# riktor/safer2-recommender

Hardware: AMD Instinct MI355X
Metric: user-solve updates/sec + sec/epoch, iALS dim=256 ml20m-shaped (higher is better)
Workload: dtype f32

## Files before the change

safer2-recommender_amd/csrc/capi.hip:

```cpp
#include <hip/hip_runtime.h>
#include <rccl/rccl.h>

#include <algorithm>
#include <climits>
#include <cmath>
#include <cstdio>
#include <cstdlib>
#include <cstring>
#include <map>
#include <random>
#include <string>
#include <thread>
#include <vector>

#include "ctx.h"
#include "wide.h"

namespace {
std::string g_last_error;
}

namespace frecsys_hip {

int fail(frecsys_ctx* c, int code, const std::string& msg) {
// ... 560 lines not shown
  if (Dp == 0)
    return fail(nullptr, FRECSYS_ERR_UNSUPPORTED,
                "dim " + std::to_string(cfg->dim) + " not supported (1..1024 built)");
  if (cfg->n_users < 0 || cfg->n_items < 0)
    return fail(nullptr, FRECSYS_ERR_INVALID, "negative entity counts");
  int cnt = 0;
  if (hipGetDeviceCount(&cnt) != hipSuccess || cnt == 0)
    return fail(nullptr, FRECSYS_ERR_NO_DEVICE, "no HIP device visible");
  auto* c = new frecsys_ctx();
  c->dim = cfg->dim;
  c->Dp = Dp;
  c->quirks = cfg->parity_quirks;
  c->n[0] = cfg->n_users;
  c->n[1] = cfg->n_items;
  if (cfg->device >= 0) {
    c->device = cfg->device;
  } else {
    (void)hipGetDevice(&c->device);
  }
  auto bail = [&](int rc) {
    g_last_error = c->err;
    frecsys_ctx_destroy(c);
    return rc;
  };
  if (hipSetDevice(c->device) != hipSuccess)
    return bail(fail(c, FRECSYS_ERR_NO_DEVICE, "hipSetDevice failed"));
  {
    int lo_pri = 0, hi_pri = 0;
    (void)hipDeviceGetStreamPriorityRange(&lo_pri, &hi_pri);
    if (hipStreamCreateWithPriority(&c->stream.h, hipStreamNonBlocking, hi_pri) != hipSuccess)
      return bail(fail(c, FRECSYS_ERR_HIP, "hipStreamCreate failed"));
  }
  if (hipEventCreate(&c->ev0.h) != hipSuccess || hipEventCreate(&c->ev1.h) != hipSuccess)
    return bail(fail(c, FRECSYS_ERR_HIP, "hipEventCreate failed"));
  const int s3_pri = 0;
  if (hipStreamCreateWithFlags(&c->stream2.h, hipStreamNonBlocking) != hipSuccess ||
      hipStreamCreateWithPriority(&c->stream3.h, hipStreamNonBlocking, s3_pri) != hipSuccess ||
      hipEventCreateWithFlags(&c->ev_fork.h, hipEventDisableTiming) != hipSuccess ||
      hipEventCreateWithFlags(&c->ev_join.h, hipEventDisableTiming) != hipSuccess ||
      hipEventCreateWithFlags(&c->ev_fork3.h, hipEventDisableTiming) != hipSuccess ||
      hipEventCreateWithFlags(&c->ev_join3.h, hipEventDisableTiming) != hipSuccess)
    return bail(fail(c, FRECSYS_ERR_HIP, "hipStreamCreate failed (stream2/3)"));
  c->stream5 = c->stream3.h;
  if (hipEventCreateWithFlags(&c->ev_pre5.h, hipEventDisableTiming) != hipSuccess ||
      hipEventCreateWithFlags(&c->ev_eager[0].h, hipEventDisableTiming) != hipSuccess ||
      hipEventCreateWithFlags(&c->ev_eager[1].h, hipEventDisableTiming) != hipSuccess)
    return bail(fail(c, FRECSYS_ERR_HIP, "hipEventCreate failed (early builds)"));
  if (const char* v = getenv("FRECSYS_DUAL")) c->dual_on = atoi(v);
  if (const char* v = getenv("FRECSYS_EAGER")) c->eager_on = atoi(v);
  if (const char* v = getenv("FRECSYS_CHOL_BASIS")) c->chol_basis_on = atoi(v);
  c->dual_max_h = Dp <= 256 ? 224 : Dp == 1024 ? 512 : 256;
  if (const char* v = getenv("FRECSYS_DUAL_MAX_H")) c->dual_max_h = atoi(v);
  if (const char* v = getenv("FRECSYS_DUAL_SERIAL")) c->dual_serial = atoi(v);
  if (const char* v = getenv("FRECSYS_SPLIT_ROWS")) c->split_rows = atoi(v);
  if (const char* v = getenv("FRECSYS_DEBUG_SKIP")) {
#ifdef FRECSYS_ABLATION
    c->debug_skip = atoi(v);
#else
    if (atoi(v) != 0)
      return bail(fail(c, FRECSYS_ERR_INVALID,
                       "FRECSYS_DEBUG_SKIP needs a -DFRECSYS_ABLATION build of libfrecsys_hip.so"));
#endif
  }
  if (const char* v = getenv("FRECSYS_WIDE_WS_MB")) c->wide_ws_mb = std::max(1, atoi(v));
  if (const char* v = getenv("FRECSYS_WIDE_PRESPLIT")) c->wide_presplit = atoi(v) != 0;
  if (const char* v = getenv("FRECSYS_WS_FREE_CAP")) c->ws_free_cap = atoi(v) != 0;
  const int max_h_cap = Dp >= 512 ? kDualWideMaxH : 32 * kDualMaxTiles;
  c->dual_max_h = std::min(c->dual_max_h, max_h_cap);
  for (int t = 0; t < 3; ++t) c->dual_max_h_side[t] = c->dual_max_h;
  if (Dp == 512 && !getenv("FRECSYS_DUAL_MAX_H"))
    c->dual_max_h_side[FRECSYS_SIDE_USER] = std::min(320, max_h_cap);
  if (const char* v = getenv("FRECSYS_DUAL_MAX_H_USER"))
    c->dual_max_h_side[0] = std::min(atoi(v), max_h_cap);
  if (const char* v = getenv("FRECSYS_DUAL_MAX_H_ITEM"))
    c->dual_max_h_side[1] = std::min(atoi(v), max_h_cap);
  for (int s = 0; s < 2; ++s) {
    const size_t rows = (size_t)std::max<int64_t>(c->n[s], 1);
    if (c->emb[s].reserve(rows * Dp) != hipSuccess ||
        c->gram[s].reserve((size_t)Dp * Dp) != hipSuccess)
      return bail(fail(c, FRECSYS_ERR_HIP, "hipMalloc failed (embeddings)"));
    (void)hipMemsetAsync(c->emb[s], 0, sizeof(float) * rows * Dp, c->stream);
    (void)hipMemsetAsync(c->gram[s], 0, sizeof(float) * Dp * Dp, c->stream);
  }
  if (c->d_fail.reserve(1) != hipSuccess || c->d_counter.reserve(1) != hipSuccess ||
      c->d_events.reserve(4) != hipSuccess)
    return bail(fail(c, FRECSYS_ERR_HIP, "hipMalloc failed"));
  (void)hipMemsetAsync(c->d_events, 0, 4 * sizeof(unsigned int), c->stream);
  c->bounds[0] = {0, c->n[0]};
  c->bounds[1] = {0, c->n[1]};
  if (hipStreamSynchronize(c->stream) != hipSuccess)
    return bail(fail(c, FRECSYS_ERR_HIP, "stream sync failed"));
  *out = c;
  return FRECSYS_OK;
}

void frecsys_ctx_destroy(frecsys_ctx* c) {
  if (!c) return;
  (void)hipSetDevice(c->device);
  for (hipStream_t s : {c->stream5, c->stream.h, c->stream2.h})
    if (s) (void)hipStreamSynchronize(s);
  if (c->comm) ncclCommDestroy(c->comm);
  delete c;
}

int frecsys_comm_unique_id(uint8_t id[128]) {
  ncclUniqueId uid;
// ... 605 lines not shown
```

safer2-recommender_amd/csrc/chol.h:

```cpp
#pragma once

#include "common.h"

constexpr int kCholYWave = 4;
constexpr int kCholWPrio = 1;

namespace frecsys_hip {

__device__ __forceinline__ float rdlane(float v, int l) {
  return __int_as_float(__builtin_amdgcn_readlane(__float_as_int(v), l));
}

typedef __attribute__((address_space(3))) float lds_float;

template <int G>
__device__ __forceinline__ void load_factor_rows(const lds_float* tile, int r, bool fl,
                                                 float (&a)[32]) {
  typedef __attribute__((address_space(3))) const f32x4v lds_f32x4c;
#pragma unroll
  for (int g = 0; g < 8; ++g) {
    const f32x4v v = *reinterpret_cast<lds_f32x4c*>(tile + r * 32 + (((g ^ (r >> 1)) & 7) << 2));
#pragma unroll
    for (int t = 0; t < 4; ++t) a[4 * g + t] = v[t];
  }
  if constexpr (G == 1) {
#pragma unroll
    for (int c = 0; c < 32; ++c) asm volatile("" : "+v"(a[c]));
  }
#pragma unroll
  for (int c = 0; c < 32; ++c) a[c] = fl ? a[c] : (c == r ? 1.0f : 0.0f);
}

__device__ __forceinline__ bool diag_factor_inv_lds_body(lds_float* tile, int lane) {
  const int r = lane & 31;
  const bool fl = lane < 32;
  float a[32];
  load_factor_rows<1>(tile, r, fl, a);
  int pmin = 0x7fffffff, pmax = 0;
#pragma unroll
  for (int k = 0; k < 32; ++k) {
    float p0 = 0.f, p1 = 0.f, p2 = 0.f, p3 = 0.f;
#pragma unroll
    for (int m = 0; m < k; m += 4) {
      const float b0 = rdlane(a[m], k);
      const float b1 = m + 1 < k ? rdlane(a[m + 1], k) : 0.0f;
      const float b2 = m + 2 < k ? rdlane(a[m + 2], k) : 0.0f;
      const float b3 = m + 3 < k ? rdlane(a[m + 3], k) : 0.0f;
      p0 += a[m] * b0;
      if (m + 1 < k) p1 += a[m + 1] * b1;
      if (m + 2 < k) p2 += a[m + 2] * b2;
      if (m + 3 < k) p3 += a[m + 3] * b3;
    }
    const float t = a[k] - ((p0 + p1) + (p2 + p3));
    const float piv = rdlane(t, k);
    const int pi = __builtin_amdgcn_readfirstlane(__float_as_int(piv));
// ... 302 lines not shown
      if (hi == 0) xvec[32 * p + lo] = x;
    }
    lds_barrier();
  }
}

typedef __attribute__((address_space(3))) int lds_int;

__device__ __forceinline__ int ld_ver(const int* f) {
  return __builtin_amdgcn_readfirstlane(*(volatile lds_int*)(f));
}
__device__ __forceinline__ void wait_ver(const int* f, int v) {
  if (ld_ver(f) < v) {
    do {
      __builtin_amdgcn_s_sleep(1);
    } while (ld_ver(f) < v);
  }
  asm volatile("" ::: "memory");
}
__device__ __forceinline__ void set_ver(int* f, int v, int lane) {
  asm volatile("s_waitcnt lgkmcnt(0)" ::: "memory");
  if (lane == 0) *(volatile lds_int*)(f) = v;
  asm volatile("" ::: "memory");
}

template <bool TR>
__device__ __forceinline__ float tile_gemv(const float* M, const float* v, int lo, int hi) {
  float s0 = 0.0f, s1 = 0.0f;
  if constexpr (!TR) {
#pragma unroll
    for (int g = 0; g < 4; ++g) {
      const f32x4v x = row_gran(M, lo, 4 * hi + g);
      const int m0 = 16 * hi + 4 * g;
      s0 += x[0] * v[m0];
      s1 += x[1] * v[m0 + 1];
      s0 += x[2] * v[m0 + 2];
      s1 += x[3] * v[m0 + 3];
    }
  } else {
#pragma unroll
    for (int m = 0; m < 16; m += 2) {
      const int m0 = 16 * hi + m;
      s0 += M[TR ? sw(m0, lo) : sw(lo, m0)] * v[m0];
      s1 += M[TR ? sw(m0 + 1, lo) : sw(lo, m0 + 1)] * v[m0 + 1];
    }
  }
  const float s = s0 + s1;
  return s + __shfl_xor(s, 32);
}

template <int T, int NW, bool BLK = true>
__device__ __forceinline__ void chol_solve_df(float* tiles, float* bvec, float* xvec,
                                              float* part, int* flag, int tid, int debug_skip,
                                              unsigned long long* prof = nullptr) {
  static_assert(NW >= 2, "one chain wave and at least one worker");
  constexpr int NT = T * (T + 1) / 2;
  constexpr bool X6 = BLK;
  constexpr bool FUSE = BLK;
  const unsigned long long t0 = prof ? clock64() : 0;
  const int lane = tid & 63, lo = lane & 31, hi = lane >> 5;
  const int wave = __builtin_amdgcn_readfirstlane(tid >> 6);
  int* ver = reinterpret_cast<int*>(part);
  int* bver = ver + NT;
  int* rcnt = bver + T;
  int* yver = rcnt + T;
  int* xver = yver + 1;
  float* rbuf = part + ((NT + 2 * T + 2 + 3) & ~3);
  if (tid < NT + 2 * T + 2) ver[tid] = 0;
  lds_barrier();

  auto trsm = [&](int I, int p) {
    float* Aip = tiles + tidx(I, p) * 1024;
    if (!FRECSYS_SKIP(debug_skip, 4)) {
      const f32x16 u = X6 ? tile_pqT_x6(Aip, tiles + tidx(p, p) * 1024, lo, hi)
                          : tile_pqT(Aip, tiles + tidx(p, p) * 1024, lo, hi);
#pragma unroll
      for (int q = 0; q < 16; ++q) Aip[sw(acc_row(q, hi), lo)] = u[q];
    }
    set_ver(ver + tidx(I, p), p + 1, lane);
  };
  auto bupd = [&](int I, int p) {
    wait_ver(bver + I, p);
    const float t = tile_gemv<false>(tiles + tidx(I, p) * 1024, bvec + 32 * p, lo, hi);
    if (hi == 0) bvec[32 * I + lo] -= t;
    set_ver(bver + I, p + 1, lane);
  };
  auto update = [&](int I, int J, int p) {
    float* Aij = tiles + tidx(I, J) * 1024;
    if (!FRECSYS_SKIP(debug_skip, 8)) {
      const float* Li = tiles + tidx(I, p) * 1024;
      const float* Lj = tiles + tidx(J, p) * 1024;
      const f32x16 u = !X6     ? tile_pqT(Li, Lj, lo, hi)
                       : I == J ? tile_pqT_x6<true>(Li, Li, lo, hi)
                                : tile_pqT_x6(Li, Lj, lo, hi);
#pragma unroll
      for (int q = 0; q < 16; ++q) Aij[sw(acc_row(q, hi), lo)] -= u[q];
    }
    set_ver(ver + tidx(I, J), p + 1, lane);
  };
  auto factor = [&](int p) {
    float* Tpp = tiles + tidx(p, p) * 1024;
    if (!FRECSYS_SKIP(debug_skip, 2)) {
      if (!diag_factor_inv<BLK>(Tpp, lane) && lane == 0) flag[0] = 1;
    }
    set_ver(ver + tidx(p, p), p + 1, lane);
  };
  auto ysolve = [&](int p) {
// ... 29 lines not shown
          if (!YW) bupd(p + 1, p);
          lap(ts);
          wait_ver(ver + tidx(p + 1, p + 1), p);
          lap(tw);
          const float* Lnp = tiles + tidx(p + 1, p) * 1024;
          f32x16 u = f32x16{0.f};
          if (!FRECSYS_SKIP(debug_skip, 8)) u = tile_pqT_x6<true>(Lnp, Lnp, lo, hi);
#pragma unroll
          for (int q = 0; q < 16; ++q) u[q] = Tnn[sw(acc_row(q, hi), lo)] - u[q];
          lap(tu);
          if (!FRECSYS_SKIP(debug_skip, 2)) ok = diag_factor_inv_acc(u, (lds_float*)Tnn);
        } else {
          if (!FRECSYS_SKIP(debug_skip, 2)) ok = diag_factor_inv_blk((lds_float*)Tnn, lane);
        }
        if (!ok && lane == 0) flag[0] = 1;
        set_ver(ver + tidx(p + 1, p + 1), p + 2, lane);
      } else {
        if (p >= 0) {
          wait_ver(ver + tidx(p + 1, p), p);
          lap(tw);
          trsm(p + 1, p);
          if (!YW) bupd(p + 1, p);
          lap(ts);
          wait_ver(ver + tidx(p + 1, p + 1), p);
          lap(tw);
          update(p + 1, p + 1, p);
          lap(tu);
        }
        factor(p + 1);
      }
      if (!YW) ysolve(p + 1);
      lap(tf);
    }
    if (prof && lane == 0) {
      atomicAdd(prof + 11, tw);
      atomicAdd(prof + 12, ts);
      atomicAdd(prof + 13, tu);
      atomicAdd(prof + 14, tf);
    }
    __builtin_amdgcn_s_setprio(0);
    if (prof && lane == 0) atomicAdd(prof + 5, clock64() - t0);
  } else if (YW && wave == YWAVE) {
#pragma unroll 1
    for (int p = 0; p < T; ++p) {
      wait_ver(ver + tidx(p, p), p + 1);
      wait_ver(bver + p, p);
      ysolve(p);
      if (p + 1 < T) {
        wait_ver(ver + tidx(p + 1, p), p + 1);
        bupd(p + 1, p);
      }
    }
  } else {
    int k = 0;
    unsigned long long tww = 0;
    auto wwait = [&](const int* f, int v) {
      if (prof) {
        const unsigned long long t = clock64();
        wait_ver(f, v);
        tww += clock64() - t;
      } else {
        wait_ver(f, v);
      }
    };
    auto wprio = [&](bool c) {
      if (c) __builtin_amdgcn_s_setprio(1);
      else __builtin_amdgcn_s_setprio(0);
    };
#pragma unroll 1
    for (int p = 0; p + 1 < T; ++p) {
#pragma unroll 1
      for (int I = p + 2; I < T; ++I, ++k) {
        if (wk_wave(k % NWK) != wave) continue;
        wwait(ver + tidx(p, p), p + 1);
        wwait(ver + tidx(I, p), p);
        wprio(I <= p + 1 + kCholWPrio);
        trsm(I, p);
        wwait(yver, p + 1);
        bupd(I, p);
      }
#pragma unroll 1
      for (int J = p + 1; J < T; ++J) {
#pragma unroll 1
        for (int I = (J == p + 1 ? p + 2 : J); I < T; ++I, ++k) {
          if (wk_wave(k % NWK) != wave) continue;
          wwait(ver + tidx(I, p), p + 1);
          wwait(ver + tidx(J, p), p + 1);
          wwait(ver + tidx(I, J), p);
          wprio(I <= p + 1 + kCholWPrio);
          update(I, J, p);
        }
      }
    }
    __builtin_amdgcn_s_setprio(0);
    if (prof && lane == 0) {
      atomicAdd(prof + 6, (clock64() - t0) / NWK);
      atomicAdd(prof + 15, tww / NWK);
    }
  }
  lds_barrier();
  if (prof && tid == 0) atomicAdd(prof + 7, clock64() - t0);

  if (wave == 0) {
    __builtin_amdgcn_s_setprio(2);
#pragma unroll 1
    for (int p = T - 1; p >= 0; --p) {
      float r = bvec[32 * p + lo];
      if (p + 1 < T) {
        wait_ver(rcnt + p, T - 2 - p);
        r = bvec[32 * p + lo] -
            tile_gemv<true>(tiles + tidx(p + 1, p) * 1024, xvec + 32 * (p + 1), lo, hi);
      }
      if (hi == 0) rbuf[lo] = r;
      wave_lds_sync();
      const float x = tile_gemv<true>(tiles + tidx(p, p) * 1024, rbuf, lo, hi);
      if (hi == 0) xvec[32 * p + lo] = x;
      set_ver(xver, T - p, lane);
    }
    __builtin_amdgcn_s_setprio(0);
  } else {
#pragma unroll 1
    for (int q = T - 1; q >= 2; --q) {
#pragma unroll 1
      for (int p = 0; p + 2 <= q; ++p) {
        if (1 + p % (NW - 1) != wave) continue;
        wait_ver(xver, T - q);
        const float t = tile_gemv<true>(tiles + tidx(q, p) * 1024, xvec + 32 * q, lo, hi);
        if (hi == 0) bvec[32 * p + lo] -= t;
        set_ver(rcnt + p, T - q, lane);
      }
    }
  }
  lds_barrier();
}

}
```

safer2-recommender_amd/csrc/ctx.h:

```cpp
#pragma once

#include <hip/hip_runtime.h>
#include <rccl/rccl.h>

#include <cstdint>
#include <map>
#include <string>
#include <vector>

#include "../../include/frecsys_hip.h"
#include "device_buf.h"
#include "kernels.h"

namespace frecsys_hip {

struct Timer {
  double total_ms = 0.0;
  int64_t launches = 0;
};

struct Work {
  double flops = 0.0, bytes = 0.0;
  int64_t entities = 0, launches = 0;
};
// ... 80 lines not shown
  std::vector<int32_t> cg_bstart;
  std::vector<int32_t> cg_iters[3];
  int64_t cg_iterations = 0, cg_unconverged = 0;
  DevBuf<float> wide_ws;
  DevBuf<char> wide_xs;
  DevBuf<char> dw_zs;
  DevBuf<float> dw_slots;
  DevBuf<float> dw_z;
  bool wide_presplit = true;
  int64_t wide_ws_mb = 16384;
  bool ws_free_cap = true;
  int64_t ws_shrinks = 0;
  int split_rows = 4096;
  std::vector<int2> h_split;
  std::vector<SplitWork> h_work;
  DevBuf<int2> d_split;
  DevBuf<SplitWork> d_work;
  DevBuf<float> d_slabs;
  std::vector<int32_t> order_h[3];
  std::vector<QueueRec> h_order[3];
  int dual_on = 1;
  uint64_t ver_counter = 0;
  uint64_t emb_ver[3] = {0, 0, 0};
  uint64_t gram_ver[2] = {0, 0};
  uint64_t gram_src[2] = {0, 0};
  uint64_t basis_gram[2] = {0, 0};
  uint64_t xrot_emb[2] = {0, 0};
  uint64_t xrot_gram[2] = {0, 0};
  uint64_t xrot_sub[2] = {0, 0};
  DevBuf<QueueRec> d_hrows[3];
  int64_t n_hrows[3] = {-1, -1, -1};
  int64_t hrows_key[3][2] = {{-1, -1}, {-1, -1}, {-1, -1}};
  struct WorkPrefix {
    bool valid = false;
    std::vector<double> h1, h2, h3;
    std::vector<int64_t> nz;
  };
  WorkPrefix wprefix[3][2];
  uint64_t hrows_gen[3] = {0, 0, 0};
  DevBuf<uint8_t> d_mark;
  bool dual_used[3] = {false, false, false};
  int eager_on = 1;
  int basis_mode[2] = {0, 0};
  float basis_mu[2] = {0.f, 0.f}, basis_lam[2] = {0.f, 0.f};
  int want_mode[2] = {0, 0};
  float want_mu[2] = {0.f, 0.f}, want_lam[2] = {0.f, 0.f};
  int chol_basis_on = 1;
  DevBuf<float> chol_work;
  bool eager_pending[2] = {false, false};
  int dual_max_h = 256;
  int dual_max_h_side[3] = {256, 256, 256};
  int dual_serial = 0;
  int debug_skip = 0;
  struct Pending {
    std::string name;
    hipEvent_t a, b;
  };
  std::vector<Pending> pending;
  std::vector<hipEvent_t> event_pool;
};

namespace frecsys_hip {

int fail(frecsys_ctx* c, int code, const std::string& msg);

#define HIP_TRY(c, expr)                                                            \
  do {                                                                              \
    hipError_t _e = (expr);                                                         \
    if (_e != hipSuccess)                                                           \
      return fail((c), FRECSYS_ERR_HIP,                                             \
                  std::string(#expr) + ": " + hipGetErrorString(_e));               \
  } while (0)

#define NCCL_TRY(c, expr)                                                           \
  do {                                                                              \
    ncclResult_t _r = (expr);                                                       \
    if (_r != ncclSuccess)                                                          \
      return fail((c), FRECSYS_ERR_RCCL,                                            \
                  std::string(#expr) + ": " + ncclGetErrorString(_r));              \
  } while (0)

void add_work(frecsys_ctx* c, const std::string& key, double flops, double bytes,
              int64_t entities);

void partition_rows(int64_t n_rows, const int64_t* row_ptr, int parts, int64_t* bounds);

template <typename T>
int ensure(frecsys_ctx* c, DevBuf<T>& b, size_t count) {
  const hipError_t e = b.reserve(count);
  if (e == hipSuccess) return FRECSYS_OK;
  return fail(c, FRECSYS_ERR_HIP,
              std::string(b ? "hipFree(*p): "
                            : "hipMalloc((void**)p, sizeof(T) * std::max<size_t>(count, 1)): ") +
                  hipGetErrorString(e));
}

#pragma GCC visibility push(hidden)

template <typename T>
int try_ensure(frecsys_ctx* c, DevBuf<T>& b, size_t count, bool* oom) {
  const hipError_t e = b.try_reserve(count, oom);
  if (e == hipSuccess) return FRECSYS_OK;
  return fail(c, FRECSYS_ERR_HIP,
              std::string(b ? "hipFree(*p): " : "hipMalloc: ") + hipGetErrorString(e));
}

// ... 82 lines not shown
```

safer2-recommender_amd/csrc/dual.hip:

```cpp
#include <hip/hip_runtime.h>

#include <cstdlib>
#include <type_traits>

#include "chol.h"
#include "common.h"
#include "kernels.h"

namespace frecsys_hip {

namespace {

constexpr int kMaxDp = 1024;

template <int HP>
__device__ __forceinline__ int dgran(int p, int g, int hh, int j) {
  return ((p * 2 + g) * 2 + hh) * HP + j;
}

template <int TH, bool BF>
struct DualCfg {
  static constexpr int HP = 32 * TH;
  static constexpr int NT = TH * (TH + 1) / 2;
  static constexpr int NW = (TH <= 4) ? 4 : 8;
// ... 314 lines not shown
        const bf16x8* zb = reinterpret_cast<const bf16x8*>(zs);
#pragma unroll
        for (int m = 0; m < MT; ++m) {
          if (valid[m]) {
#pragma unroll
            for (int g = 0; g < 2; ++g) {
              bf16x8 av[3], bv[3];
#pragma unroll
              for (int p = 0; p < 3; ++p) {
                av[p] = zb[dgran<HP>(p, g, hi, aoff[m])];
                bv[p] = zb[dgran<HP>(p, g, hi, boff[m])];
              }
              acc[m] = mfma_x6(av, bv, acc[m]);
            }
          }
        }
      } else {
#pragma unroll
        for (int m = 0; m < MT; ++m) {
          if (valid[m]) {
#pragma unroll
            for (int s = 0; s < 16; ++s) {
              const float* zr = zs + (2 * s + hi) * HP;
              acc[m] = mfma32(zr[aoff[m]], zr[boff[m]], acc[m]);
            }
          }
        }
      }
    }
    if (!RDS && c + 1 < NC) store_slab(next, (c + 1) & 1);
    lds_barrier();
  };
  for (int c = 0; c < NC; c += 2) {
    slab_step(c, ra, rb);
    if (c + 1 < NC) slab_step(c + 1, rb, ra);
  }

#pragma unroll
  for (int m = 0; m < MT; ++m) {
    if (valid[m]) {
      const int I = (aoff[m] - lo) >> 5, J = (boff[m] - lo) >> 5;
      float* tile = tiles + tidx(I, J) * 1024;
#pragma unroll
      for (int q = 0; q < 16; ++q) {
        const int i = acc_row(q, hi);
        const bool dg = (32 * I + i) == (32 * J + lo);
        tile[sw(i, lo)] = acc[m][q] + (dg ? 1.0f : 0.0f);
      }
    }
  }
  lds_barrier();
  mark(1);
  chol_solve_df<TH, NW, (TH >= kDualBlkTH)>(tiles, bvec, xvec, part, flag, tid, a.debug_skip,
                                            a.prof);
  mark(2);

  {
    const int D4 = Dp >> 2, R = NTHR / D4;
    const int c4 = tid % D4, g = tid / D4;
    float* red = tiles;
    float4 acc4 = make_float4(0.f, 0.f, 0.f, 0.f);
    if (g < R && !FRECSYS_SKIP(a.debug_skip, 64)) {
      for (int j0 = g; j0 < ntot; j0 += 8 * R) {
        float4 rv[8];
        float wv[8];
#pragma unroll
        for (int u = 0; u < 8; ++u) {
          const int j = j0 + u * R;
          rv[u] = make_float4(0.f, 0.f, 0.f, 0.f);
          wv[u] = 0.0f;
          if (j < ntot) {
            wv[u] = cvec[j] * xvec[j];
            rv[u] = *reinterpret_cast<const float4*>(a.Xrot + (int64_t)ids[j] * Dp + 4 * c4);
          }
        }
#pragma unroll
        for (int u = 0; u < 8; ++u) {
          acc4.x += wv[u] * rv[u].x;
          acc4.y += wv[u] * rv[u].y;
          acc4.z += wv[u] * rv[u].z;
          acc4.w += wv[u] * rv[u].w;
        }
      }
      *reinterpret_cast<float4*>(red + g * Dp + 4 * c4) = acc4;
    }
    lds_barrier();
    for (int i = tid; i < Dp; i += NTHR) {
      float v = 0.0f;
      for (int gg = 0; gg < R; ++gg) v += red[gg * Dp + i];
      a.out_rot[blk_v(a.pos0 + blockIdx.x, i, Dp)] = v;
    }
  }
  mark(3);
  if (a.prof && tid == 0) atomicAdd(a.prof + 4, 1ull);
  if (tid == 0 && flag[0]) atomicMin(a.fail, (unsigned long long)(e + 1));
}


__device__ __forceinline__ void wave_sync() { wave_lds_sync(); }

template <int T>
__device__ __forceinline__ void chol_solve_wave(float* tiles, float* bvec, float* xvec,
                                                int* flag, int lane, int debug_skip) {
  const int lo = lane & 31, hi = lane >> 5;
  float y[T];
#pragma unroll
  for (int p = 0; p < T; ++p) {
// ... 710 lines not shown
```

safer2-recommender_amd/csrc/kernels.h:

```cpp
#pragma once

#include <hip/hip_runtime.h>
#include <stdint.h>

#include <vector>

namespace frecsys_hip {

struct QueueRec {
  int32_t entity;
  int32_t h;
  int64_t p0;
};

struct SplitWork {
  int32_t pos;
  int32_t k0;
  int32_t k1;
  int32_t slab;
};

struct SolveArgs {
  int kind;
  int quirk;
  const int64_t* row_ptr;
  const int32_t* col;
  int64_t row_lo;
  int64_t n_rows;
  const QueueRec* order;
  unsigned int* counter;
  const float* X;
  int64_t n_other;
  const float* G;
  const float* E;
  float* out;
  float reg, reg_exp, w, alpha, eta;
  int lambda_is_reg;
  const float* entity_weight;
  const float* entity_reg;
  const float* other_weight;
  unsigned long long* fail;
  int debug_skip;
  unsigned long long* prof;
  const int2* split;
  int64_t n_split;
  float* slabs;
  const SplitWork* work;
  int64_t n_work;
  const char* xsplit;
};

constexpr int kGramGroups = 16;
struct GramPlan {
  int64_t n = 0;
  int64_t rpl = 0;
  int64_t nleaf = 0;
  int ngroup = 0;
  size_t slab_floats = 0;
};
GramPlan gram_plan(int Dp, int64_t n);
inline int64_t gram_group_leaf(const GramPlan& p, int g) {
  return p.ngroup ? (int64_t)g * p.nleaf / p.ngroup : 0;
}
inline void gram_owned_groups(const GramPlan& p, int world, int rank, int* lo, int* hi) {
  *lo = (int)((int64_t)p.ngroup * rank / world);
  *hi = (int)((int64_t)p.ngroup * (rank + 1) / world);
}
size_t gram_leaf_floats(const GramPlan& p, int g_lo, int g_hi);

struct GramArgs {
  const float* X;
  const float* w;
  float* partials;
  float* gslabs;
  GramPlan plan;
  int g_lo, g_hi;
  int64_t row0;
  int64_t n;
};

struct LossArgs {
  const int64_t* row_ptr;
  const int32_t* col;
  int64_t row_lo, n_rows;
  const float* U;
  const float* V;
  const float* G;
  float beta;
  int half;
  float* out;
  float* quad;
  int quad_parts;
  void* gsplit;
  int raw;
  hipEvent_t ev_gather;
};


struct DualArgs {
  int kind;
  int quirk;
  int Dp;
  const QueueRec* order;
  int64_t n_rows;
  const int32_t* col;
  const float* Xrot;
  const float* tdiag;
  const float* toff;
  int unit_m;
  const float* basis_status;
  int64_t n_other;
  float* out_rot;
  float* table;
  int64_t pos0;
  float reg, reg_exp, w, alpha;
  int lambda_is_reg;
  const float* entity_weight;
  const float* entity_reg;
  const float* other_weight;
  unsigned long long* fail;
  int debug_skip;
  unsigned long long* prof;
};

constexpr int kDualMaxTiles = 8;

constexpr int kCgE = 16;
constexpr int kCgU = 8;
constexpr int kCgCoopRows = 256;
constexpr int kCgBatchRows = 4096;
struct CgArgs {
  int kind;
  int quirk;
  int Dp, dim;
  const QueueRec* order;
  const int32_t* bstart;
  int64_t n_batches;
  const int32_t* col;
  const float* X;
  int64_t n_other;
  const float* G;
  float* out;
  float reg, reg_exp, w, alpha;
  int lambda_is_reg;
  const float* entity_weight;
  const float* entity_reg;
  const float* other_weight;
  int max_iter;
  float tol;
  int32_t* iters;
  unsigned long long* stats;
  unsigned long long* fail;
};
size_t cg_lds_bytes(int Dp);
void cg_plan_batches(const QueueRec* order, int64_t n, std::vector<int32_t>* bstart);
hipError_t launch_cg(const CgArgs& a, hipStream_t s);

constexpr int kExplainGroup = 32;
constexpr int kExplainChunk = 256;
constexpr int kExplainMaxTop = 32;
struct ExplainArgs {
  int kind;
  int Dp;
  const int64_t* row_ptr;
  const int32_t* col;
  const int64_t* qrows;
  int64_t r0, n;
  const int64_t* tgt_ptr;
  const int32_t* tgt;
  int64_t tgt_base;
  const int64_t* coff;
  const int32_t* prow;
  const int32_t* order;
  const float* X;
// ... 273 lines not shown
```

safer2-recommender_amd/csrc/solve.hip:

```cpp
#include <hip/hip_runtime.h>

#include <type_traits>

#include "chol.h"
#include "common.h"
#include "kernels.h"

constexpr int kSyrkSB = 1;

namespace frecsys_hip {

namespace {

constexpr int kRing = 4;

template <int T, bool BF>
struct TiledCfg {
  static constexpr int Dp = 32 * T;
  static constexpr int NT = T * (T + 1) / 2;
  static constexpr int NW = (T <= 2) ? 4 : 8;
  static constexpr int NTHR = NW * 64;
  static constexpr int MT = (NT + NW - 1) / NW;
  static constexpr int R = BF ? 32 : ((T <= 2) ? 16 : (T >= 8 ? 64 : 32));
  static constexpr int NSLOT = R * Dp / 4;
// ... 508 lines not shown
          }
        }
      }
      if (tid < Dp) {
#pragma unroll 4
        for (int r = 0; r < R; ++r) bacc += ring_bw[slot * R + r] * st[r * Dp + tid];
      }
      if (more) store_stage(buf ^ 1, c + 1);
      if (ring_more) ring_store(c + 2, nid, nsa, nbw);
      lds_barrier();
    }
    store_tiles();
  }
  mark(1);
  if constexpr (BF) {
    if (bown && bg == 1) part[bc] = bpart;
    lds_barrier();
    if (tid < Dp) bacc += bpart + part[tid];
    lds_barrier();
  }
  mark(9);

  if (PARTIAL) {
    if (tid < Dp) a.slabs[(size_t)slab0 * slab_floats + NT * 1024 + tid] = bacc;
    return;
  }

  mark(10);
  if (tid < Dp) {
    float b = bacc;
    if (is_u_kind(kind)) b *= us;
    bvec[tid] = b;
  }
  lds_barrier();
  mark(2);

  if (grad) {
    if (tid < Dp) {
      const int i = tid, I = i >> 5, ri = i & 31;
      float y = 0.0f;
      for (int j = 0; j < Dp; ++j) {
        float aij;
        if (j <= i)
          aij = tiles[tidx(I, j >> 5) * 1024 + sw(ri, j & 31)];
        else
          aij = cvar_upper(kind, a.G[i * Dp + j], a.w, omega);
        y += aij * xvec[j];
      }
      a.out[e * Dp + i] = xvec[i] - a.eta * (y - bvec[i]);
    }
    return;
  }

  chol_solve_df<T, NW>(tiles, bvec, xvec, part, flag, tid, a.debug_skip, a.prof);
  mark(3);
  if (tid < Dp) a.out[e * Dp + tid] = xvec[tid];
  if (tid == 0 && flag[0]) atomicMin(a.fail, (unsigned long long)(e + 1));
  if (a.prof && tid == 0) {
    atomicAdd(a.prof + 4, 1ull);
    atomicAdd(a.prof + 8, (unsigned long long)ntot);
  }
}

__device__ __forceinline__ void wave_sync() {
  __builtin_amdgcn_fence(__ATOMIC_RELEASE, "wavefront");
  __builtin_amdgcn_wave_barrier();
  __builtin_amdgcn_fence(__ATOMIC_ACQUIRE, "wavefront");
}

template <int Dp>
__global__ void __launch_bounds__(256) solve_small_kernel(SolveArgs a) {
  constexpr int WPB = 4, CH = 64, PER = Dp * Dp / 64;
  __shared__ float sA[WPB][Dp * Dp];
  __shared__ float sX[WPB][CH * Dp];
  __shared__ float sB[WPB][Dp];
  __shared__ float sE[WPB][Dp];
  __shared__ float sSA[WPB][CH];
  __shared__ float sBW[WPB][CH];
  const int wave = threadIdx.x >> 6, lane = threadIdx.x & 63;
  const int64_t idx = (int64_t)blockIdx.x * WPB + wave;
  if (idx >= a.n_rows) return;
  const int64_t e = a.row_lo + idx;
  const int64_t p0 = a.row_ptr[e];
  const int64_t h = a.row_ptr[e + 1] - p0;
  if (h == 0) return;
  const int kind = a.kind;
  const bool vk = is_v_kind(kind);
  int64_t extra = 0;
  if (vk && a.quirk && h > 128 && (h % 128) != 0) extra = 128 - (h % 128);
  const int64_t ntot = h + extra;
  float acc[PER];
#pragma unroll
  for (int t = 0; t < PER; ++t) acc[t] = 0.0f;
  float bacc = 0.0f;
  float* X = sX[wave];
  for (int64_t c0 = 0; c0 < ntot; c0 += CH) {
    const int64_t k = c0 + lane;
    int id = -1;
    float sa = 0.f, bw = 0.f;
    if (k < ntot) {
      id = a.col[p0 + virt_pos(k, h)];
      if (vk) {
        const float nu = a.other_weight[id];
        sa = sqrtf(nu);
        bw = (k < h) ? nu : 0.0f;
      } else {
        sa = 1.0f;
// ... 209 lines not shown
```

safer2-recommender_amd/csrc/train.hip:

```cpp
#include <algorithm>
#include <climits>
#include <cstdio>
#include <cstdlib>
#include <string>
#include <vector>

#include "ctx.h"
#include "wide.h"

namespace {

const char* const kSolveNames[3] = {"solve_user", "solve_item", "solve_eval"};

bool is_vkind(int kind) { return kind == FRECSYS_KIND_WEIGHTED_V || kind == FRECSYS_KIND_CVAR_GRAD_V; }
bool is_ukind(int kind) { return kind == FRECSYS_KIND_WEIGHTED_U || kind == FRECSYS_KIND_CVAR_GRAD_U; }
bool is_grad(int kind) { return kind == FRECSYS_KIND_CVAR_GRAD_U || kind == FRECSYS_KIND_CVAR_GRAD_V; }

double dspace_solve_flops(double d) { return d * d * d / 3.0 + 2.0 * d * d; }

bool dual_prof_on() {
  static const bool on = getenv("FRECSYS_DUAL_PROF") != nullptr;
  return on;
}
int prof_counters(frecsys_ctx* c, DevBuf<unsigned long long>& buf, size_t n,
// ... 229 lines not shown
  }
  if (is_vkind(p->kind)) {
    rc = upload(c, c->d_entity_reg, p->entity_reg, (size_t)c->n[side]);
    if (rc) return rc;
    rc = upload(c, c->d_other_weight, p->other_weight, (size_t)c->n[other]);
    if (rc) return rc;
  }
  HIP_TRY(c, hipMemsetAsync(c->d_fail, 0xFF, sizeof(unsigned long long), c->stream));
  return FRECSYS_OK;
}

int end_solve(frecsys_ctx* c, int side, bool gather, unsigned long long* f) {
  HIP_TRY(c, hipMemcpyAsync(f, c->d_fail, sizeof(*f), hipMemcpyDeviceToHost, c->stream));
  if (gather && side < 2 && (c->world > 1 || c->comm)) {
    ScopedTimer t(c, "allgather");
    int rc = allgather_rows(c, c->emb[side], side, c->Dp);
    if (rc) return rc;
    t.stop();
  }
  HIP_TRY(c, hipStreamSynchronize(c->stream));
  flush_ktimers(c);
  return FRECSYS_OK;
}

SolveArgs solve_args(frecsys_ctx* c, int side, const frecsys_solve_params* p) {
  const int other = side == 1 ? 0 : 1;
  int64_t lo, hi;
  shard(c, side, &lo, &hi);
  SolveArgs a{};
  a.kind = p->kind;
  a.order = c->d_order[side];
  a.counter = c->d_counter;
  a.quirk = c->quirks;
  a.row_ptr = c->rp[side];
  a.col = c->col[side];
  a.row_lo = lo;
  a.n_rows = hi - lo;
  a.X = p->from_snapshot ? c->snap[other] : c->emb[other];
  a.n_other = c->n[other];
  a.G = c->gram[other];
  a.E = c->emb[side];
  a.out = c->emb[side];
  a.reg = p->reg;
  a.reg_exp = p->reg_exp;
  a.w = p->unobserved_weight;
  a.alpha = p->alpha;
  a.eta = p->stepsize;
  a.lambda_is_reg = p->lambda_is_reg;
  a.entity_weight = (is_ukind(p->kind) && p->entity_weight) ? c->d_entity_weight.dev.get() : nullptr;
  a.entity_reg = is_vkind(p->kind) ? c->d_entity_reg.dev.get() : nullptr;
  a.other_weight = is_vkind(p->kind) ? c->d_other_weight.dev.get() : nullptr;
  a.fail = c->d_fail;
  a.debug_skip = c->debug_skip;
  return a;
}

bool hspace_allowed(const frecsys_ctx* c, int side, const frecsys_solve_params* p) {
  const int other = side == 1 ? 0 : 1;
  bool m_spd = p->reg > 0.0f && p->unobserved_weight >= 0.0f;
  if (m_spd && is_ukind(p->kind) && p->entity_weight)
    for (int64_t i = 0; i < c->n[side] && m_spd; ++i) m_spd = p->entity_weight[i] >= 0.0f;
  if (m_spd && is_vkind(p->kind) && !p->lambda_is_reg) {
    const float base = p->alpha * p->unobserved_weight * (float)c->n[other];
    for (int64_t i = 0; i < c->n[side] && m_spd; ++i) m_spd = p->entity_reg[i] + base > 0.0f;
  }
  return m_spd;
}

struct SidePlan {
  bool dual = false;
  int64_t n_dspace = 0, n_nonempty = 0;
  int bmode = 0;
  float bmu = 0.f, blam = 0.f;
  std::string pre;
};
SidePlan plan_side(const frecsys_ctx* c, int side, const frecsys_solve_params* p, int64_t n_rows,
                   bool force_dspace) {
  const bool vq = is_vkind(p->kind);
  SidePlan pl;
  pl.pre = kSolveNames[side];
  pl.dual = c->dual_on && !force_dspace && hspace_allowed(c, side, p) && !is_grad(p->kind) &&
            c->Dp >= 64 && c->dual_max_h_side[side] > 0 &&
            (int64_t)c->order_h[side].size() == c->order_n[side];
  pl.n_dspace = pl.dual ? first_le(c, side, vq, c->dual_max_h_side[side]) : n_rows;
  pl.n_nonempty = pl.dual ? first_le(c, side, vq, 0) : n_rows;
  if (c->chol_basis_on && p->kind == FRECSYS_KIND_IALS &&
      (p->lambda_is_reg || p->reg_exp == 0.0f)) {
    pl.bmode = 1;
    pl.bmu = p->unobserved_weight;
    pl.blam = p->reg;
  }
  return pl;
}

DualArgs dual_args(const frecsys_ctx* c, int side, const SolveArgs& a, const SidePlan& pl) {
  const int other = side == 1 ? 0 : 1;
  DualArgs d{};
  d.kind = a.kind;
  d.quirk = c->quirks;
  d.Dp = c->Dp;
  d.col = a.col;
  d.Xrot = c->xrot[other];
  d.tdiag = c->tri[other];
  d.toff = c->tri[other] + c->Dp;
  d.unit_m = pl.bmode;
  d.basis_status = c->tri[other];
  d.n_other = a.n_other;
  d.reg = a.reg;
  d.reg_exp = a.reg_exp;
  d.w = a.w;
  d.alpha = a.alpha;
  d.lambda_is_reg = a.lambda_is_reg;
  d.entity_weight = a.entity_weight;
  d.entity_reg = a.entity_reg;
  d.other_weight = a.other_weight;
  d.fail = a.fail;
  d.debug_skip = a.debug_skip;
  return d;
}

int launch_hspace_wide_bucket(frecsys_ctx* c, const SolveArgs& a, const SidePlan& pl, DualArgs d,
                              int64_t lo, int64_t hi) {
  const size_t per = dual_wide_zs_bytes(c->Dp) + sizeof(float) * (dual_wide_slot_floats() + 512);
  const size_t held = c->dw_zs.cap() + sizeof(float) * (c->dw_slots.cap() + c->dw_z.cap());
  int64_t nbat =
      std::max<int64_t>(1, std::min<int64_t>(hi - lo, (int64_t)(ws_budget(c, held) / per)));
  if (hi <= lo) return FRECSYS_OK;
  int rc = ensure_batch(c, c->dw_zs, dual_wide_zs_bytes(c->Dp), &nbat);
  if (rc) return rc;
  rc = ensure_batch(c, c->dw_slots, dual_wide_slot_floats(), &nbat);
  if (rc) return rc;
  rc = ensure_batch(c, c->dw_z, (size_t)512, &nbat);
  if (rc) return rc;
  d.prof = nullptr;
  for (int64_t b0 = lo; b0 < hi; b0 += nbat) {
    d.order = a.order + b0;
    d.n_rows = std::min(nbat, hi - b0);
    d.pos0 = b0 - pl.n_dspace;
    HIP_TRY(c, launch_dual_wide(d, c->dw_zs, c->dw_slots, c->dw_z, a.fail, c->stream));
  }
  return FRECSYS_OK;
}

int launch_hspace(frecsys_ctx* c, int side, const SolveArgs& a, const SidePlan& pl) {
  const int other = side == 1 ? 0 : 1;
  const bool vq = is_vkind(a.kind);
  const int64_t n_dspace = pl.n_dspace, n_nonempty = pl.n_nonempty;
  DualArgs d = dual_args(c, side, a, pl);
  unsigned long long* prof = nullptr;
  int rc = prof_counters(c, c->dual_prof, 16 * 9, &prof);
  if (rc) return rc;
  const int64_t n_hs = n_nonempty - n_dspace;
  const size_t n_blk = (size_t)((n_hs + 63) / 64) * 64;
  rc = ensure(c, c->dual_table, n_blk * 3 * c->Dp);
  if (rc) return rc;
  rc = ensure(c, c->out_rot[side], n_blk * c->Dp);
  if (rc) return rc;
  d.out_rot = c->out_rot[side];
  size_t k = ktimer_begin(c, pl.pre + ".hspace", c->stream);
  d.order = a.order + n_dspace;
  d.n_rows = n_hs;
  d.table = c->dual_table;
  d.pos0 = 0;
  HIP_TRY(c, launch_dual_ldl(d, c->stream));
  const bool two_lanes = !c->dual_serial;
  if (two_lanes) {
    HIP_TRY(c, hipEventRecord(c->ev_fork3, c->stream));
    HIP_TRY(c, hipStreamWaitEvent(c->stream3, c->ev_fork3, 0));
  }
  int64_t lo = n_dspace;
// ... 30 lines not shown
    const double ne = (double)n_hs;
    add_work(c, pl.pre + ".hspace", hsum.h2 * dd + hsum.h3 / 3.0 + 4.0 * hsum.h1 * dd,
             (2.0 * dd * 4.0 + 4.0) * hsum.h1 + ne * (8.0 + 3.0 * dd * 4.0 + dd * 4.0), n_hs);
  }
  k = ktimer_begin(c, pl.pre + ".rotate", c->stream);
  HIP_TRY(c, launch_rotate(c->out_rot[side], a.order + n_dspace, 0, n_hs, c->qsplit[other][1],
                           a.out, c->Dp, c->stream, 1));
  ktimer_end(c, k, c->stream);
  return FRECSYS_OK;
}

int launch_mixed(frecsys_ctx* c, int side, const SolveArgs& a, const SidePlan& pl) {
  const int other = side == 1 ? 0 : 1;
  hipStream_t s2 = c->dual_serial ? c->stream : c->stream2;
  if (pl.n_dspace > 0) HIP_TRY(c, hipEventRecord(c->ev_fork, c->stream));
  c->want_mode[other] = pl.bmode;
  c->want_mu[other] = pl.bmu;
  c->want_lam[other] = pl.blam;
  const QueueRec* hrows = nullptr;
  int64_t nhrows = 0;
  uint64_t hsub = 0;
  int rc = hspace_rows(c, side, other, pl.n_dspace, pl.n_nonempty, &hrows, &nhrows, &hsub);
  if (rc) return rc;
  const size_t k = ktimer_begin(c, pl.pre + ".basis", c->stream);
  rc = prepare_basis(c, other, a.X, c->stream, pl.bmode, pl.bmu, pl.blam, hrows, nhrows, hsub);
  if (rc) return rc;
  ktimer_end(c, k, c->stream);
  if (pl.n_dspace > 0) {
    HIP_TRY(c, hipStreamWaitEvent(s2, c->ev_fork, 0));
    SolveArgs ap = a;
    ap.n_rows = pl.n_dspace;
    rc = launch_dspace(c, side, ap, s2, pl.pre, true);
    if (rc) return rc;
    HIP_TRY(c, hipEventRecord(c->ev_join, s2));
  }
  rc = launch_hspace(c, side, a, pl);
  if (rc) return rc;
  if (pl.n_dspace > 0) HIP_TRY(c, hipStreamWaitEvent(c->stream, c->ev_join, 0));
  return FRECSYS_OK;
}

int print_dual_prof(frecsys_ctx* c, int side) {
  unsigned long long hp[16 * 9];
  int rc = prof_readback(c, c->dual_prof, 16 * 9, hp);
  if (rc) return rc;
  for (int t = 1; t <= 8; ++t) {
    const unsigned long long n = hp[16 * t + 4];
    if (!n) continue;
    fprintf(stderr, "[dual-prof] side %d tiles %d n %llu cycles/entity: setup %.0f slabs %.0f chol %.0f "
            "yz %.0f | chain %.0f workers %.0f factored %.0f\n", side, t, n,
            (double)hp[16 * t] / n, (double)hp[16 * t + 1] / n, (double)hp[16 * t + 2] / n,
            (double)hp[16 * t + 3] / n, (double)hp[16 * t + 5] / n, (double)hp[16 * t + 6] / n,
            (double)hp[16 * t + 7] / n);
  }
  return FRECSYS_OK;
}

int solve_side(frecsys_ctx* c, int32_t side, const frecsys_solve_params* p, bool force_dspace);

int solve_verdict(frecsys_ctx* c, int side, const frecsys_solve_params* p, const SidePlan& pl,
                  unsigned long long f) {
  if (f == ~0ull) return FRECSYS_OK;
  if (c->debug_skip) return FRECSYS_OK;
  if (pl.dual && ((side < 2 && c->comm) || pl.n_dspace < pl.n_nonempty)) {
    ++c->hspace_reruns;
    return solve_side(c, side, p, true);
  }
  c->err_entity = (int64_t)f - 1;
  return fail(c, FRECSYS_ERR_NOT_SPD,
              "LLT failed (matrix not SPD) for entity " + std::to_string(c->err_entity));
}

int solve_side(frecsys_ctx* c, int32_t side, const frecsys_solve_params* p, bool force_dspace) {
  if (!c || !valid_side(side) || !p) return fail(c, FRECSYS_ERR_INVALID, "solve: bad arguments");
  int rc = check_solve_args(c, "solve: ", side, p);
  if (rc) return rc;
  rc = begin_solve(c, side, p, side < 2 ? 1 << side : 0);
  if (rc) return rc;
  rc = build_order(c, side);
  if (rc) return rc;
  const SolveArgs a = solve_args(c, side, p);
  const SidePlan pl = plan_side(c, side, p, a.n_rows, force_dspace);
  c->dual_used[side] = pl.dual;
  if (side < 2) emb_written(c, side);
  {
    ScopedTimer t(c, kSolveNames[side]);
    if (pl.dual && pl.n_dspace < pl.n_nonempty) {
      rc = launch_mixed(c, side, a, pl);
    } else {
      rc = launch_dspace(c, side, a, c->stream, pl.pre,
                         c->Dp >= 32 && (int64_t)c->order_h[side].size() == c->order_n[side],
                         c->dual_serial ? nullptr : c->stream2);
    }
    if (rc) return rc;
    t.stop();
  }
  if (side < 2 && c->comm) {
    NCCL_TRY(c, ncclAllReduce(c->d_fail, c->d_fail, 1, ncclUint64, ncclMin, c->comm, c->stream));
  }
  unsigned long long f = ~0ull;
  rc = end_solve(c, side, true, &f);
  if (rc) return rc;
  if (dual_prof_on() && pl.dual && c->dual_prof) {
    rc = print_dual_prof(c, side);
    if (rc) return rc;
  }
// ... 324 lines not shown
```

Measured before the change: 9.490 million.

## Use precomputed per-wave task schedule for blocked Cholesky worker waves

Replaces the round-robin assignment of TRSM and trailing-update tile tasks to worker waves with a compile-time per-wave task list for the T=8, NW=8 case. The lists are ordered so that critical-path tiles run earlier, which is meant to cut worker stalls on version flags in the dataflow Cholesky. The old round-robin order is kept as a table and selectable through the FRECSYS_CHOL_SCHED environment variable. Risks are a bad static order that deadlocks or stalls, and reliance on the table matching the wave layout. It also adds a profiling printout of chain-wave timings.

```diff
diff --git a/safer2-recommender_amd/csrc/capi.hip b/safer2-recommender_amd/csrc/capi.hip
--- a/safer2-recommender_amd/csrc/capi.hip
+++ b/safer2-recommender_amd/csrc/capi.hip
@@ -636,6 +636,7 @@
   c->dual_max_h = Dp <= 256 ? 224 : Dp == 1024 ? 512 : 256;
   if (const char* v = getenv("FRECSYS_DUAL_MAX_H")) c->dual_max_h = atoi(v);
   if (const char* v = getenv("FRECSYS_DUAL_SERIAL")) c->dual_serial = atoi(v);
+  if (const char* v = getenv("FRECSYS_CHOL_SCHED")) c->chol_sched = atoi(v) != 0;
   if (const char* v = getenv("FRECSYS_SPLIT_ROWS")) c->split_rows = atoi(v);
   if (const char* v = getenv("FRECSYS_DEBUG_SKIP")) {
 #ifdef FRECSYS_ABLATION
diff --git a/safer2-recommender_amd/csrc/chol.h b/safer2-recommender_amd/csrc/chol.h
--- a/safer2-recommender_amd/csrc/chol.h
+++ b/safer2-recommender_amd/csrc/chol.h
@@ -1,6 +1,7 @@
 #pragma once
 
 #include "common.h"
+#include "chol_sched.h"
 
 constexpr int kCholYWave = 4;
 constexpr int kCholWPrio = 1;
@@ -409,7 +410,7 @@
 template <int T, int NW, bool BLK = true>
 __device__ __forceinline__ void chol_solve_df(float* tiles, float* bvec, float* xvec,
                                               float* part, int* flag, int tid, int debug_skip,
-                                              unsigned long long* prof = nullptr) {
+                                              bool sched, unsigned long long* prof = nullptr) {
   static_assert(NW >= 2, "one chain wave and at least one worker");
   constexpr int NT = T * (T + 1) / 2;
   constexpr bool X6 = BLK;
@@ -545,7 +546,6 @@
       }
     }
   } else {
-    int k = 0;
     unsigned long long tww = 0;
     auto wwait = [&](const int* f, int v) {
       if (prof) {
@@ -560,28 +560,52 @@
       if (c) __builtin_amdgcn_s_setprio(1);
       else __builtin_amdgcn_s_setprio(0);
     };
-#pragma unroll 1
-    for (int p = 0; p + 1 < T; ++p) {
-#pragma unroll 1
-      for (int I = p + 2; I < T; ++I, ++k) {
-        if (wk_wave(k % NWK) != wave) continue;
-        wwait(ver + tidx(p, p), p + 1);
-        wwait(ver + tidx(I, p), p);
-        wprio(I <= p + 1 + kCholWPrio);
-        trsm(I, p);
-        wwait(yver, p + 1);
-        bupd(I, p);
-      }
-#pragma unroll 1
-      for (int J = p + 1; J < T; ++J) {
-#pragma unroll 1
-        for (int I = (J == p + 1 ? p + 2 : J); I < T; ++I, ++k) {
+    auto strsm = [&](int I, int p) {
+      wwait(ver + tidx(p, p), p + 1);
+      wwait(ver + tidx(I, p), p);
+      wprio(I <= p + 1 + kCholWPrio);
+      trsm(I, p);
+      wwait(yver, p + 1);
+      bupd(I, p);
+    };
+    auto supd = [&](int I, int J, int p) {
+      wwait(ver + tidx(I, p), p + 1);
+      wwait(ver + tidx(J, p), p + 1);
+      wwait(ver + tidx(I, J), p);
+      wprio(I <= p + 1 + kCholWPrio);
+      update(I, J, p);
+    };
+    using Sched = CholSched<T, NW>;
+    if constexpr (Sched::kHas) {
+      static_assert(Sched::kSlots == NWK, "a table of another wave layout");
+      const int slot = YW ? wave - 1 - (wave > YWAVE ? 1 : 0) : wave - 1;
+      const unsigned short* list = sched ? Sched::kTask[slot] : Sched::kRrTask[slot];
+      const int n = sched ? Sched::kLen[slot] : Sched::kRrLen[slot];
+      unsigned nxt = list[0];
+#pragma unroll 1
+      for (int i = 0; i < n; ++i) {
+        const unsigned e = nxt;
+        nxt = list[i + 1];
+        const int I = (e >> 8) & 15, J = (e >> 4) & 15, p = e & 15;
+        if (e >> 12) supd(I, J, p);
+        else strsm(I, p);
+      }
+    } else {
+      int k = 0;
+#pragma unroll 1
+      for (int p = 0; p + 1 < T; ++p) {
+#pragma unroll 1
+        for (int I = p + 2; I < T; ++I, ++k) {
           if (wk_wave(k % NWK) != wave) continue;
-          wwait(ver + tidx(I, p), p + 1);
-          wwait(ver + tidx(J, p), p + 1);
-          wwait(ver + tidx(I, J), p);
-          wprio(I <= p + 1 + kCholWPrio);
-          update(I, J, p);
+          strsm(I, p);
+        }
+#pragma unroll 1
+        for (int J = p + 1; J < T; ++J) {
+#pragma unroll 1
+          for (int I = (J == p + 1 ? p + 2 : J); I < T; ++I, ++k) {
+            if (wk_wave(k % NWK) != wave) continue;
+            supd(I, J, p);
+          }
         }
       }
     }
diff --git a/safer2-recommender_amd/csrc/chol_sched.h b/safer2-recommender_amd/csrc/chol_sched.h
--- /dev/null
+++ b/safer2-recommender_amd/csrc/chol_sched.h
@@ -0,0 +1,36 @@
+#pragma once
+
+namespace frecsys_hip {
+
+constexpr unsigned short kCholSchedEnd = 0xffff;
+
+template <int T, int NW>
+struct CholSched {
+  static constexpr bool kHas = false;
+};
+
+template <>
+struct CholSched<8, 8> {
+  static constexpr bool kHas = true;
+  static constexpr int kSlots = 6, kMax = 17;
+  static constexpr int kLen[6] = {17, 16, 17, 16, 16, 16};
+  static constexpr unsigned short kTask[6][18] = {
+      {0x0200, 0x1210, 0x1610, 0x0311, 0x1321, 0x1621, 0x1730, 0x1631, 0x1532, 0x1551, 0x1750, 0x0733, 0x1553, 0x1761, 0x1663, 0x1763, 0x1765, 0xffff},
+      {0x0300, 0x1310, 0x1420, 0x0411, 0x1421, 0x0422, 0x0622, 0x1731, 0x1641, 0x1542, 0x1651, 0x1760, 0x1752, 0x0744, 0x1754, 0x1774, 0xffff, 0xffff},
+      {0x0400, 0x1220, 0x1330, 0x0511, 0x1331, 0x1630, 0x1531, 0x1432, 0x1740, 0x1650, 0x1660, 0x1742, 0x1643, 0x1662, 0x1753, 0x1664, 0x1775, 0xffff},
+      {0x0500, 0x1410, 0x1710, 0x0611, 0x1521, 0x1431, 0x1441, 0x1640, 0x1442, 0x1732, 0x0633, 0x1543, 0x1652, 0x0644, 0x1654, 0x1764, 0xffff, 0xffff},
+      {0x0600, 0x1510, 0x1520, 0x1430, 0x1720, 0x1440, 0x0522, 0x1550, 0x1541, 0x0533, 0x1642, 0x1751, 0x1770, 0x1653, 0x1762, 0x1773, 0xffff, 0xffff},
+      {0x0700, 0x1320, 0x1620, 0x0711, 0x1530, 0x1721, 0x1540, 0x0722, 0x1632, 0x1741, 0x1552, 0x1661, 0x1743, 0x1771, 0x1772, 0x0755, 0xffff, 0xffff},
+  };
+  static constexpr int kRrLen[6] = {17, 17, 16, 16, 16, 16};
+  static constexpr unsigned short kRrTask[6][18] = {
+      {0x0200, 0x1210, 0x1220, 0x1330, 0x1540, 0x1660, 0x0611, 0x1721, 0x1441, 0x1751, 0x0622, 0x1442, 0x1752, 0x0733, 0x1753, 0x1654, 0x1765, 0xffff},
+      {0x0300, 0x1310, 0x1320, 0x1430, 0x1640, 0x1760, 0x0711, 0x1331, 0x1541, 0x1661, 0x0722, 0x1542, 0x1662, 0x1543, 0x1663, 0x1754, 0x1775, 0xffff},
+      {0x0400, 0x1410, 0x1420, 0x1530, 0x1740, 0x1770, 0x1321, 0x1431, 0x1641, 0x1761, 0x1432, 0x1642, 0x1762, 0x1643, 0x1763, 0x1664, 0xffff, 0xffff},
+      {0x0500, 0x1510, 0x1520, 0x1630, 0x1550, 0x0311, 0x1421, 0x1531, 0x1741, 0x1771, 0x1532, 0x1742, 0x1772, 0x1743, 0x1773, 0x1764, 0xffff, 0xffff},
+      {0x0600, 0x1610, 0x1620, 0x1730, 0x1650, 0x0411, 0x1521, 0x1631, 0x1551, 0x0422, 0x1632, 0x1552, 0x0533, 0x1553, 0x0644, 0x1774, 0xffff, 0xffff},
+      {0x0700, 0x1710, 0x1720, 0x1440, 0x1750, 0x0511, 0x1621, 0x1731, 0x1651, 0x0522, 0x1732, 0x1652, 0x0633, 0x1653, 0x0744, 0x0755, 0xffff, 0xffff},
+  };
+};
+
+}
diff --git a/safer2-recommender_amd/csrc/ctx.h b/safer2-recommender_amd/csrc/ctx.h
--- a/safer2-recommender_amd/csrc/ctx.h
+++ b/safer2-recommender_amd/csrc/ctx.h
@@ -156,6 +156,7 @@
   int dual_max_h_side[3] = {256, 256, 256};
   int dual_serial = 0;
   int debug_skip = 0;
+  int chol_sched = 1;
   struct Pending {
     std::string name;
     hipEvent_t a, b;
diff --git a/safer2-recommender_amd/csrc/dual.hip b/safer2-recommender_amd/csrc/dual.hip
--- a/safer2-recommender_amd/csrc/dual.hip
+++ b/safer2-recommender_amd/csrc/dual.hip
@@ -390,7 +390,7 @@
   lds_barrier();
   mark(1);
   chol_solve_df<TH, NW, (TH >= kDualBlkTH)>(tiles, bvec, xvec, part, flag, tid, a.debug_skip,
-                                            a.prof);
+                                            a.chol_sched != 0, a.prof);
   mark(2);
 
   {
diff --git a/safer2-recommender_amd/csrc/kernels.h b/safer2-recommender_amd/csrc/kernels.h
--- a/safer2-recommender_amd/csrc/kernels.h
+++ b/safer2-recommender_amd/csrc/kernels.h
@@ -41,6 +41,7 @@
   const float* other_weight;
   unsigned long long* fail;
   int debug_skip;
+  int chol_sched;
   unsigned long long* prof;
   const int2* split;
   int64_t n_split;
@@ -120,6 +121,7 @@
   const float* other_weight;
   unsigned long long* fail;
   int debug_skip;
+  int chol_sched;
   unsigned long long* prof;
 };
 
diff --git a/safer2-recommender_amd/csrc/solve.hip b/safer2-recommender_amd/csrc/solve.hip
--- a/safer2-recommender_amd/csrc/solve.hip
+++ b/safer2-recommender_amd/csrc/solve.hip
@@ -584,7 +584,8 @@
     return;
   }
 
-  chol_solve_df<T, NW>(tiles, bvec, xvec, part, flag, tid, a.debug_skip, a.prof);
+  chol_solve_df<T, NW>(tiles, bvec, xvec, part, flag, tid, a.debug_skip, a.chol_sched != 0,
+                       a.prof);
   mark(3);
   if (tid < Dp) a.out[e * Dp + tid] = xvec[tid];
   if (tid == 0 && flag[0]) atomicMin(a.fail, (unsigned long long)(e + 1));
diff --git a/safer2-recommender_amd/csrc/train.hip b/safer2-recommender_amd/csrc/train.hip
--- a/safer2-recommender_amd/csrc/train.hip
+++ b/safer2-recommender_amd/csrc/train.hip
@@ -305,6 +305,7 @@
   a.other_weight = is_vkind(p->kind) ? c->d_other_weight.dev.get() : nullptr;
   a.fail = c->d_fail;
   a.debug_skip = c->debug_skip;
+  a.chol_sched = c->chol_sched;
   return a;
 }
 
@@ -369,6 +370,7 @@
   d.other_weight = a.other_weight;
   d.fail = a.fail;
   d.debug_skip = a.debug_skip;
+  d.chol_sched = a.chol_sched;
   return d;
 }
 
@@ -505,6 +507,11 @@
             (double)hp[16 * t] / n, (double)hp[16 * t + 1] / n, (double)hp[16 * t + 2] / n,
             (double)hp[16 * t + 3] / n, (double)hp[16 * t + 5] / n, (double)hp[16 * t + 6] / n,
             (double)hp[16 * t + 7] / n);
+    if (hp[16 * t + 14])
+      fprintf(stderr, "[dual-prof] side %d tiles %d chain: waits %.0f trsm %.0f update %.0f factor %.0f "
+              "| worker waits %.0f\n", side, t, (double)hp[16 * t + 11] / n,
+              (double)hp[16 * t + 12] / n, (double)hp[16 * t + 13] / n, (double)hp[16 * t + 14] / n,
+              (double)hp[16 * t + 15] / n);
   }
   return FRECSYS_OK;
 }
```

Result: faster. 9.720 million (median of 6 runs) (+2.4%).
